# leggedrobotics/open3d_slam_private

Measured on AMD Instinct MI355X. Metric: ICP iterations/sec (scan-to-map), higher is better.
Workload: dtype f32

## Files before the change

include/o3dslam_reg_debug.h:

```cpp
#ifndef O3DSLAM_REG_DEBUG_H
#define O3DSLAM_REG_DEBUG_H

#include "o3dslam_reg.h"

#ifdef __cplusplus
extern "C" {
#endif

typedef struct {
    int32_t struct_size;
    int32_t profile_loop;
    int32_t match_variant;
    int32_t debug_flags;
    int32_t disable_halo;
    int32_t lanes_per_point;
    int32_t disable_fused;
    int32_t reserved;
} reg_debug_params;

REG_API reg_status reg_debug_configure(reg_handle* h, const reg_debug_params* d);

REG_API reg_status reg_debug_halo_bound(reg_handle* h, const float* xyz, int64_t n, float* out);

REG_API reg_status reg_debug_halo_witness(reg_handle* h, const float* xyz, int64_t n, int32_t* out);

REG_API reg_status reg_debug_live_resources(int64_t out[4]);

#ifdef __cplusplus
}
#endif
#endif
```

open3d_slam_private_amd/capi.py:

```python
from __future__ import annotations

import ctypes as C
import math
import os
import subprocess
import weakref

import numpy as np

_HERE = os.path.dirname(os.path.abspath(__file__))
_SO = os.environ.get("O3D_REG_LIB") or os.path.join(_HERE, "lib", "libo3dslam_reg.so")

STATUS_NAMES = {0: "OK", 1: "EMPTY_TARGET", 2: "EMPTY_SOURCE", 3: "NO_CORRESPONDENCES", 4: "BAD_TRANSFORM",
                5: "NOT_CONFIGURED", 6: "BAD_ARGUMENT", 7: "MISSING_FIELD", 8: "DEVICE_ERROR", 9: "UNSUPPORTED",
                10: "OUT_OF_BOUNDS"}
OUT_OF_BOUNDS = 10
COST_P2PL, COST_GICP = 0, 1
COST_O3D_P2PL, COST_O3D_P2P = 2, 3
SMOOTH_LEN_MAX = 15


class RegError(RuntimeError):
    def __init__(self, status, msg=""):
        self.status = status
# ... 344 lines not shown
PM_POINT_TO_PLANE, PM_POINT_TO_POINT = 0, 1
ROBUST_FCTS = {"cauchy": 0, "welsch": 1, "sc": 2, "gm": 3, "tukey": 4, "huber": 5, "L1": 6, "student": 7}
SCALE_ESTIMATORS = {"none": 0, "mad": 1, "berg": 2, "std": 3}
DISTANCE_TYPES = {"point2point": 0, "point2plane": 1}


EXPORTS = ["reg_default_params", "reg_shipped_params", "reg_create", "reg_destroy", "reg_last_error",
           "reg_set_stream", "reg_set_target", "reg_set_source", "reg_register", "reg_compute", "reg_prepare",
           "reg_linearize", "reg_get_correspondences", "reg_match_local", "reg_trim_histogram", "reg_reduce_local",
           "reg_solve_update", "reg_host_solve6", "reg_host_x_to_T", "reg_host_centroid", "reg_get_target_info", "reg_profile_kernels", "reg_source_centroid_sums", "reg_prepare_centroid", "reg_compose",
           "reg_dist_begin", "reg_dist_buffers", "reg_dist_phase", "reg_dist_finish",
           "reg_dist_fused_buffers", "reg_dist_poll", "reg_estimate_normals", "reg_smooth_normals", "reg_host_solve6_xicp",
           "reg_set_target_f64", "reg_get_target_source_indices", "reg_voxelize_within_volume", "reg_carve_indices", "reg_dist_xicp_buffers", "reg_dist_gather_buffers",
           "reg_dist_record", "reg_dist_centroid_sums", "reg_dist_prepare",
           "reg_information_matrix", "reg_set_source_f64", "reg_debug_configure", "reg_debug_halo_bound", "reg_debug_halo_witness",
           "reg_debug_live_resources",
           "reg_dist_get_unique_id", "reg_dist_init", "reg_dist_init_custom", "reg_dist_register", "reg_dist_shutdown",
           "reg_dist_info", "reg_dist_steer_create", "reg_dist_steer_destroy", "reg_dist_steer_step",
           "reg_dist_steer_counts", "reg_host_tail_plan", "reg_host_o3d_update",
           "reg_default_pm_chain", "reg_check_pm_chain", "reg_set_pm_chain", "reg_get_robust_state",
           "reg_get_correspondences_k", "reg_host_robust_weights", "reg_host_pm_p2p_update",
           "reg_get_var_trim", "reg_host_var_trim",
           "reg_get_covariance", "reg_get_covariance_sums", "reg_host_censi_covariance", "reg_get_minimizer_stats",
           "reg_get_degeneracy", "reg_get_bound", "reg_host_solution_remap",
           "reg_default_ternary_xicp", "reg_check_ternary_xicp", "reg_set_ternary_xicp", "reg_get_ternary_xicp",
           "reg_host_ternary_decide", "reg_host_partial_constraint", "reg_host_solve6_xicp_rhs",
           "reg_default_ssn_params", "reg_sampling_surface_normal", "reg_filter_points",
           "reg_default_octree_params", "reg_octree_grid", "reg_host_octree_root", "reg_host_octree_random_picks",
           "reg_filter_cloud", "reg_host_glibc_rand", "reg_default_voxel_grid_params", "reg_voxel_grid",
           "reg_overlap_indices", "reg_set_pair_overlap_f64", "reg_get_source_source_indices",
           "reg_compute_fpfh", "reg_match_features", "reg_ransac_correspondences", "reg_host_ransac_est_k",
# ... 27 lines not shown
        return _lib
    if not os.path.exists(_SO):
        raise ImportError(f"{_SO} is missing: build it with `python -c 'import __graft_entry__ as g; g.build()'` "
                          "(hipcc --offload-arch=gfx950).  There is no CPU fallback for the registration path.")
    lib = C.CDLL(_SO)
    vp, i64, f32p = C.c_void_p, C.c_int64, C.c_void_p
    lib.reg_create.argtypes = [C.POINTER(RegParams), C.POINTER(vp)]
    lib.reg_destroy.argtypes = [vp]
    lib.reg_last_error.argtypes = [vp]
    lib.reg_last_error.restype = C.c_char_p
    lib.reg_set_stream.argtypes = [vp, vp]
    lib.reg_debug_configure.argtypes = [vp, C.POINTER(RegDebugParams)]
    lib.reg_debug_halo_bound.argtypes = [vp, f32p, i64, f32p]
    lib.reg_debug_halo_witness.argtypes = [vp, f32p, i64, vp]
    lib.reg_debug_live_resources.argtypes = [C.POINTER(C.c_int64)]
    lib.reg_dist_get_unique_id.argtypes = [C.c_char_p]
    lib.reg_dist_init.argtypes = [vp, C.c_char_p, C.c_int, C.c_int]
    lib.reg_dist_init_custom.argtypes = [vp, C.POINTER(Collectives), C.c_int, C.c_int]
    lib.reg_dist_register.argtypes = [vp, f32p, f32p, C.POINTER(RegResult)]
    lib.reg_dist_shutdown.argtypes = [vp]
    lib.reg_dist_info.argtypes = [vp, C.POINTER(C.c_int64), C.POINTER(C.c_int32), C.POINTER(C.c_int32), C.POINTER(C.c_int32)]
    lib.reg_dist_steer_create.argtypes = [C.c_int, C.c_int, C.c_int, C.c_float, C.c_int]
    lib.reg_dist_steer_create.restype = vp
    lib.reg_dist_steer_destroy.argtypes = [vp]
    lib.reg_dist_steer_destroy.restype = None
    lib.reg_dist_steer_step.argtypes = [vp, C.POINTER(DistReply)]
    lib.reg_dist_steer_step.restype = DistAction
    lib.reg_dist_steer_counts.argtypes = [vp, C.POINTER(C.c_int32), C.POINTER(C.c_int32), C.POINTER(C.c_int32)]
    lib.reg_dist_steer_counts.restype = None
    lib.reg_set_source_f64.argtypes = [vp, vp, vp, vp, i64, C.c_int]
# ... 1390 lines not shown


def host_solve6_xicp(A, b, flags):
    x = np.zeros(6, np.float32)
    f = np.ascontiguousarray(flags, np.int32)
    rank = load_library().reg_host_solve6_xicp(_ptr(_f32(A).reshape(36)), _ptr(_f32(b)), _ptr(f), _ptr(x))
    return x, rank


def host_x_to_T(x):
    T = np.zeros(16, np.float32)
    load_library().reg_host_x_to_T(_ptr(_f32(x)), _ptr(T))
    return _T_out(T)


def host_centroid(xyz):
    xyz = _f32(xyz)
    out = np.zeros(3, np.float32)
    load_library().reg_host_centroid(_ptr(xyz), xyz.shape[1], xyz.shape[0], _ptr(out))
    return out


def host_o3d_update(cost, sums):
    s = np.ascontiguousarray(sums, np.float64).reshape(32)
    U = np.zeros(16, np.float64)
    rank = C.c_int32()
    st = load_library().reg_host_o3d_update(int(cost), _ptr(s), _ptr(U), C.byref(rank))
    if st != 0:
        raise RegError(st, "reg_host_o3d_update")
    return U.reshape(4, 4).T.copy(), rank.value
# ... 32 lines not shown
```

open3d_slam_private_amd/csrc/host_dist.hpp:

```cpp
#pragma once
#include <thread>

struct Deadline {
    std::chrono::steady_clock::time_point t_end;
    explicit Deadline(double seconds) : t_end(std::chrono::steady_clock::now() + std::chrono::duration_cast<std::chrono::steady_clock::duration>(std::chrono::duration<double>(seconds))) {}
    bool expired() const { return std::chrono::steady_clock::now() > t_end; }
};

static reg_status dist_stream_wait(reg_handle* h, double timeout_s, const char* what) {
    const Deadline dl(timeout_s);
    for (unsigned spins = 0;; ++spins) {
        const hipError_t e = hipStreamQuery(h->stream);
        if (e == hipSuccess) return REG_OK;
        if (e != hipErrorNotReady) {
            h->err = std::string(what) + ": " + hipGetErrorString(e);
            return REG_DEVICE_ERROR;
        }
        if ((spins & 63) == 63) {
            if (dl.expired()) {
                h->err = std::string(what) + ": the stream did not drain within the deadline (O3D_DIST_TIMEOUT_S): a peer died or a "
                                              "collective never completed";
                return REG_DEVICE_ERROR;
            }
            std::this_thread::sleep_for(std::chrono::microseconds(50));
// ... 430 lines not shown

int reg_host_solve6(const float A[36], const float b[6], float x[6]) { return solve6_p2pl(A, b, x); }

int reg_host_solve6_xicp(const float A[36], const float b[6], const int32_t flags[6], float x[6]) {
    int f[6];
    for (int k = 0; k < 6; ++k) f[k] = flags[k];
    return solve6_xicp(A, b, f, x);
}

void reg_host_x_to_T(const float x[6], float T[16]) {
    float Tr[16];
    x_to_T(x, Tr);
    row_to_col(Tr, T);
}

reg_status reg_host_o3d_update(int cost, const double sums[32], double T_update[16], int32_t* rank) {
    if (!cost_is_o3d(cost) || !sums || !T_update) return REG_BAD_ARGUMENT;
    if (sums[28] == 0.0) return REG_NO_CORRESPONDENCES;
    double U[16];
    const int r = o3d_update(cost == REG_COST_O3D_P2P, sums, U);
    for (int i = 0; i < 4; ++i)
        for (int j = 0; j < 4; ++j) T_update[4 * j + i] = U[4 * i + j];
    if (rank) *rank = r;
    return REG_OK;
}

void reg_host_centroid(const float* xyz, int64_t stride, int64_t n, float out[3]) {
    long long s[3] = {0, 0, 0};
    for (int64_t i = 0; i < n; ++i)
        for (int k = 0; k < 3; ++k) s[k] += llrint((double)xyz[i * stride + k] * 65536.0);
// ... 5 lines not shown
```

open3d_slam_private_amd/csrc/host_math.hpp:

```cpp
#pragma once
#include <cmath>
#include <cstdint>
#include <cstring>

#if defined(__HIPCC__)
#include <hip/hip_runtime.h>
#define O3D_HD __host__ __device__
#else
#define O3D_HD
#endif

namespace o3dreg {

O3D_HD inline void m4_identity(float* T) {
    memset(T, 0, 16 * sizeof(float));
    T[0] = T[5] = T[10] = T[15] = 1.f;
}

O3D_HD inline void m4_mul(const float* A, const float* B, float* C) {
    float R[16];
    for (int i = 0; i < 4; ++i)
        for (int j = 0; j < 4; ++j) {
            float s = A[4 * i] * B[j];
            float t = A[4 * i + 1] * B[4 + j];
            s = s + t;
            t = A[4 * i + 2] * B[8 + j];
            s = s + t;
            t = A[4 * i + 3] * B[12 + j];
            s = s + t;
            R[4 * i + j] = s;
        }
    memcpy(C, R, sizeof(R));
}

O3D_HD inline float float_from_orderable(uint32_t k) {
    const uint32_t u = (k & 0x80000000u) ? (k & 0x7fffffffu) : ~k;
    float v;
    memcpy(&v, &u, 4);
    return v;
}

O3D_HD inline void m4_transpose(const float* A, float* B) {
    float R[16];
    for (int i = 0; i < 4; ++i)
        for (int j = 0; j < 4; ++j) R[4 * i + j] = A[4 * j + i];
    memcpy(B, R, sizeof(R));
// ... 835 lines not shown
```

open3d_slam_private_amd/csrc/kernels_tail.hpp:

```cpp
#pragma once

#ifndef O3D_TAIL_ACQ
#define O3D_TAIL_ACQ 0
#endif
#ifndef O3D_TAIL_THREADS
#define O3D_TAIL_THREADS 512
#endif
constexpr int kTailThreads = O3D_TAIL_THREADS;
#ifndef O3D_TAIL_SLOTS
#define O3D_TAIL_SLOTS 1024
#endif
#ifndef O3D_TAIL_WGS_PER_CU
#define O3D_TAIL_WGS_PER_CU 1
#endif
constexpr int kTailSlots = O3D_TAIL_SLOTS;
constexpr int kTailWgsPerCu = O3D_TAIL_WGS_PER_CU;
constexpr int kTailPts = kTailSlots / kTailThreads;
constexpr int kTailRec = 12;
constexpr int kTailHistRow = 32;
constexpr int kTailCoarse = 256;
constexpr int kTailMaxIters = 64;
constexpr int kTailSyncWords = 256;
constexpr int kTailRing = 4;
constexpr int kTailBandCntWord = 128;
// ... 74 lines not shown
}
__device__ __forceinline__ void tail_st_f64(double* p, double x) {
    __hip_atomic_store(reinterpret_cast<unsigned long long*>(p), (unsigned long long)__double_as_longlong(x), __ATOMIC_RELAXED,
                       __HIP_MEMORY_SCOPE_AGENT);
}
__device__ __forceinline__ unsigned long long tail_ld_u64(const void* p) {
    return __hip_atomic_load(reinterpret_cast<unsigned long long*>(const_cast<void*>(p)), __ATOMIC_RELAXED, __HIP_MEMORY_SCOPE_AGENT);
}
__device__ __forceinline__ void tail_st_u64(void* p, unsigned long long x) {
    __hip_atomic_store(reinterpret_cast<unsigned long long*>(p), x, __ATOMIC_RELAXED, __HIP_MEMORY_SCOPE_AGENT);
}
__device__ __forceinline__ unsigned tail_ld_u32(const unsigned* p) {
    return __hip_atomic_load(const_cast<unsigned*>(p), __ATOMIC_RELAXED, __HIP_MEMORY_SCOPE_AGENT);
}

__device__ __noinline__ __attribute__((flatten)) void tail_solve_update(IterState* sit, const double* tot, const uint32_t* misc, float* s_x, UpdWork* work,
                                               bool trim, unsigned n_band_raw, unsigned n_band_all) {
    const int lane = (int)(threadIdx.x & 63);
    const float r_limit_last = sit->limit_last, r_limit_sel = __uint_as_float(misc[2]);
    const int r_dbg_narrow = sit->debug_narrow_band & 1;
    const int r_fixed = sit->fixed_iters, r_iters = sit->iterations;
    const int r_xnc = sit->xicp_nc;
    const double r_tot28 = tot[28];
    float r_T[16];
#pragma unroll
    for (int i = 0; i < 16; ++i) r_T[i] = sit->T[i];
    const int r = lane >> 3, c = lane & 7;
    double a = 0.0;
    if (r < 6 && c < 7) {
        if (c < 6) {
            const int lo = r < c ? r : c, hi = r < c ? c : r;
            const int k = lo * 6 - (lo * (lo - 1)) / 2 + (hi - lo);
            a = (double)(float)tot[k];
        } else {
            a = (double)(-(float)tot[21 + r]);
        }
    }
    const double a_orig = a;
    double dmax = 0.0;
#pragma unroll
    for (int j = 0; j < 6; ++j) dmax = fmax(dmax, fabs(__shfl(a_orig, j * 8 + j)));
    bool well = dmax > 0.0;
    const double piv_thr = 1e-4 * dmax;
#pragma unroll
    for (int j = 0; j < 6; ++j) {
        const double pj = __shfl(a, j * 8 + j);
        well = well && (pj > piv_thr);
        const double ajc = __shfl(a, j * 8 + c);
        const double arj = __shfl(a, r * 8 + j);
        const double qd = ajc / pj;
        a = (r == j) ? qd : a - arj * qd;
    }
    double xsol[6];
#pragma unroll
    for (int i = 0; i < 6; ++i) xsol[i] = __shfl(a, i * 8 + 6);
    if (lane != 0) return;
    const float limit = r_limit_sel;
    const float r_limit_prev = sit->limit_prev;
    sit->limit_prev2 = r_limit_prev;
    sit->limit_prev = r_limit_last;
    sit->limit_last = limit;
    {
        const Band nb = trim ? predict_band(limit, r_limit_last, r_limit_prev, n_band_all, sit->band_lo, sit->band_hi, r_dbg_narrow)
                             : Band{INFINITY, INFINITY};
        sit->band_lo = nb.lo;
        sit->band_hi = nb.hi;
    }
    sit->band_count = n_band_raw;
    sit->stall = 0;
    if (r_tot28 == 0.0) {
        sit->status = REG_NO_CORRESPONDENCES;
        sit->done = 1;
        return;
    }
    float x[6], dT[16], Tn[16];
    int rank = 6;
    if (r_xnc > 0) {
        rank = upd_solve6_xicp_inl(tot, sit->xicp_flags, s_x, work);
        for (int i = 0; i < 6; ++i) x[i] = s_x[i];
    } else if (well) {
        for (int i = 0; i < 6; ++i) x[i] = (float)xsol[i];
    } else {
        rank = upd_solve6_p2pl_inl(tot, s_x, work);
        for (int i = 0; i < 6; ++i) x[i] = s_x[i];
    }
    sit->rank_last = rank;
    x_to_T(x, dT);
    m4_mul(dT, r_T, Tn);
    for (int i = 0; i < 16; ++i) sit->T_prev[i] = r_T[i];
    for (int i = 0; i < 16; ++i) sit->T[i] = Tn[i];
    sit->iterations = r_iters + 1;
    bool iterate;
    if (r_fixed > 0)
        iterate = r_iters + 1 < r_fixed;
    else
        iterate = sit->chk.check(sit->T);
    if (!iterate) sit->done = 1;
}

__device__ __forceinline__ void tail_gicp_factor(const Xf& T, const float4 s, const float4 a0, const float4 a1, const float4 q,
                                                 const float4 b0, const float4 b1, float d2, double (&v)[kSums]) {
    const float3 tp = xf_point(T, s.x, s.y, s.z);
    const double r[3] = {(double)q.x - (double)tp.x, (double)q.y - (double)tp.y, (double)q.z - (double)tp.z};
    const double Cp[9] = {a0.x, a0.y, a0.z, a0.y, a0.w, a1.x, a0.z, a1.x, a1.y};
    const double Cq[9] = {b0.x, b0.y, b0.z, b0.y, b0.w, b1.x, b0.z, b1.x, b1.y};
    double R[9];
#pragma unroll
    for (int a = 0; a < 3; ++a)
#pragma unroll
        for (int c = 0; c < 3; ++c) R[3 * a + c] = (double)T.m[4 * a + c];
    double RC[9], S[9];
#pragma unroll
// ... 796 lines not shown
                }
                wave_reduce32(v);
                if ((lane & 1) == 0) sh[wave][lane >> 1] = v[0];
                __syncthreads();
                if (t < kSums) {
                    double v2 = 0.0;
#pragma unroll
                    for (int w2 = 0; w2 < kWaves; ++w2) v2 += sh[w2][t];
                    tot[t] += v2;
                }
                __syncthreads();
            }
        }
        TAIL_STAMP(10);
        if (t < kSums) sit->sums[t] = tot[t];
        if (wave == 0) {
            if (kGicp)
                tail_solve_update_gicp(sit, tot, reinterpret_cast<double*>(s_x), work);
            else
                tail_solve_update(sit, tot, misc, s_x, work, trim, n_band_raw, wide ? misc[12] : n_band_raw);
        }
        __syncthreads();
        TAIL_STAMP(11);
        if (sit->done) {
            exit_reason = 1;
            ++k_local;
            break;
        }
        if (k_local + 1 >= cfg.max_iters) {
            exit_reason = 3;
            ++k_local;
            break;
        }
    }
    if (exit_reason == 2 || exit_reason == 4) {
// ... 80 lines not shown
    uint32_t* hw = reinterpret_cast<uint32_t*>(host);
    for (int w2 = lane; w2 < kMirrorWords; w2 += 64) hw[w2] = mir_w[w2];
    HostMirror::SeqRecord* srec = &host->ring[cfg.seq % kSeqRing];
    {
        const HostMirror* m = reinterpret_cast<const HostMirror*>(mir_w);
        uint32_t word = 0;
        if (lane == 2) word = (uint32_t)m->iterations;
        if (lane == 3) word = (uint32_t)m->done;
        if (lane == 4) word = (uint32_t)m->stall;
        if (lane == 6) word = __float_as_uint(m->limit_last);
        if (lane == 7) word = __float_as_uint(m->limit_prev);
        if (lane >= 2 && lane < 8) reinterpret_cast<uint32_t*>(srec)[lane] = word;
    }
    __threadfence_system();
    if (lane == 0) {
        __hip_atomic_store(&srec->seq, cfg.seq, __ATOMIC_RELEASE, __HIP_MEMORY_SCOPE_SYSTEM);
        __hip_atomic_store(&host->seq, cfg.seq, __ATOMIC_RELEASE, __HIP_MEMORY_SCOPE_SYSTEM);
    }
}
```

open3d_slam_private_amd/csrc/kernels_update.hpp:

```cpp
#pragma once

__global__ void __launch_bounds__(64)
k_pack_contrib(double* __restrict__ acc, const IterState* __restrict__ it, float* __restrict__ contrib) {
    const int c = threadIdx.x;
    double* hdr = reinterpret_cast<double*>(contrib);
    if (it->done || it->stall) {
        if (c < kSums) hdr[c] = 0.0;
        if (c == 0) reinterpret_cast<uint32_t*>(contrib)[64] = 0u;
        return;
    }
    if (c < kSums) {
        double t = 0;
        for (int r = 0; r < kAccRows; ++r) {
            t += acc[(size_t)r * kSums + c];
            acc[(size_t)r * kSums + c] = 0.0;
        }
        hdr[c] = t;
    }
    if (c == 0) reinterpret_cast<uint32_t*>(contrib)[64] = it->band_count;
}

__device__ __forceinline__ void lds_barrier() {
    asm volatile("s_waitcnt lgkmcnt(0)" ::: "memory");
    __builtin_amdgcn_s_barrier();
// ... 80 lines not shown
            dst[3 * kk + rr] = sacc + a2;
        }
}

template <bool kP2P, int kWg>
__device__ __noinline__ __attribute__((flatten)) int upd_o3d(const double* tot, double* U_out, UpdWork* w) {
    double s[kSums], U[16];
    for (int i = 0; i < kSums; ++i) s[i] = tot[i];
    const int rank = kP2P ? o3d_update_p2p(s, U) : o3d_update_p2pl_in(s, U, w->sym.s);
    for (int i = 0; i < 16; ++i) U_out[i] = U[i];
    return rank;
}

enum UpdPath { kUpdGeneric = 0, kUpdSelect, kUpdFused, kUpdGathered, kUpdFinish };
constexpr int kUpdLeanThreads = 512;
constexpr int upd_threads(UpdPath p) { return (p == kUpdSelect || p == kUpdFinish) ? kUpdLeanThreads : 1024; }

template <bool kO3d, UpdPath kPath>
__device__ __forceinline__ void reduce_update_body(const double* __restrict__ partials, int n_blocks, IterState* it,
                                                   HostMirror* host, unsigned long long seq, int fused_arg,
                                                   const float* __restrict__ band, float* __restrict__ w_out,
                                                   const SelectState* __restrict__ sel, const float* __restrict__ gathered_arg,
                                                   int n_ranks, int my_rank, XicpState* __restrict__ xs) {
    constexpr int kThreads = upd_threads(kPath);
    constexpr bool kBand = kPath == kUpdGeneric || kPath == kUpdFused || kPath == kUpdGathered;
    static_assert(!kBand || kThreads == 1024, "the band code is written for 1024 threads");
    const bool finish = kPath == kUpdGeneric ? fused_arg == 2 : kPath == kUpdFinish;
    const int fused = kPath == kUpdGeneric ? (fused_arg == 1 ? 1 : 0) : ((kPath == kUpdFused || kPath == kUpdGathered) ? 1 : 0);
    const float* __restrict__ const gathered = (kPath == kUpdGeneric || kPath == kUpdGathered) ? gathered_arg : nullptr;
    const int contrib_cap = contrib_cap_for(n_ranks);
    const size_t contrib_stride = contrib_floats(contrib_cap);
    __shared__ double sh[32][kSums];
    __shared__ double tot[kSums];
    __shared__ uint32_t hist[2048 + 64];
    __shared__ uint32_t wave_tot[16];
    __shared__ uint32_t pick[2];
    __shared__ float s_limit;
    __shared__ uint32_t bd2[kBandCap];
    constexpr int kDirectCap = 256;
    __shared__ __attribute__((aligned(16))) uint32_t bdk[kDirectCap];
// ... 8 lines not shown
    __shared__ double s_dl[6];
    __shared__ __attribute__((aligned(16))) unsigned char s_work[kUpdWorkBytes];
    UpdWork* const work = reinterpret_cast<UpdWork*>(s_work);
    constexpr int kStateWords = (int)(sizeof(IterState) / 4);
    static_assert(sizeof(IterState) % 4 == 0 && kStateWords <= 1024, "IterState must be a whole number of words");
    __shared__ __attribute__((aligned(16))) uint32_t s_state[kStateWords];
    IterState* const sit = reinterpret_cast<IterState*>(s_state);
    constexpr int kPer = 1024 / kThreads;
    static_assert(kPer == 1 || kPer % 2 == 0, "the parts are combined in pairs");
    const int comp = threadIdx.x & (kSums - 1), part = threadIdx.x / kSums;
    for (int w = threadIdx.x; w < kStateWords; w += kThreads) s_state[w] = reinterpret_cast<const uint32_t*>(it)[w];
    double t = 0;
    double tp[kPer];
#pragma unroll
    for (int j = 0; j < kPer; ++j) tp[j] = 0;
    if constexpr (kPer > 1) {
        if (!finish) {
            for (int r0 = 0; r0 < n_blocks; r0 += 32 * 8) {
                double v[kPer][8];
#pragma unroll
                for (int j = 0; j < kPer; ++j)
#pragma unroll
                    for (int u = 0; u < 8; ++u) {
                        const int b = r0 + kPer * part + j + 32 * u;
                        v[j][u] = partials[(size_t)(b < n_blocks ? b : 0) * kSums + comp];
                    }
#pragma unroll
                for (int j = 0; j < kPer; ++j)
                    if (r0 + kPer * part + j < n_blocks) {
#pragma unroll
                        for (int u = 0; u < 8; ++u) tp[j] += (r0 + kPer * part + j + 32 * u < n_blocks) ? v[j][u] : 0.0;
                    }
            }
        }
    } else if (!gathered && !finish) {
        const int n_rows = fused ? kAccRows : n_blocks;
        for (int b0 = part; b0 < n_rows; b0 += 32 * 8) {
            double v8[8];
#pragma unroll
            for (int u = 0; u < 8; ++u) {
                const int b = b0 + 32 * u;
                v8[u] = partials[(size_t)(b < n_rows ? b : part) * kSums + comp];
            }
#pragma unroll
            for (int u = 0; u < 8; ++u) t += (b0 + 32 * u < n_rows) ? v8[u] : 0.0;
        }
    }
// ... 70 lines not shown
    if (gathered) {
        for (int r = part; r < n_ranks; r += 32)
            t += reinterpret_cast<const double*>(gathered + (size_t)r * contrib_stride)[comp];
    } else if (fused) {
        for (int b = part; b < kAccRows; b += 32)
            const_cast<double*>(partials)[(size_t)b * kSums + comp] = 0.0;
    }
    if constexpr (kPer > 1) {
#pragma unroll
        for (int j = 0; j < kPer / 2; ++j) sh[(kPer / 2) * part + j][comp] = tp[2 * j] + tp[2 * j + 1];
    } else {
        t += __shfl_xor(t, 32);
        if ((threadIdx.x & 63) < 32) sh[threadIdx.x >> 6][comp] = t;
    }
    if (threadIdx.x == 0) {
        s_limit = INFINITY;
    }
    lds_barrier();
    if (threadIdx.x < kSums) {
        double s = 0;
#pragma unroll
        for (int p = 0; p < 16; ++p) s += sh[p][threadIdx.x];
        tot[threadIdx.x] = finish ? sit->sums[threadIdx.x] : s;
    }
    if (threadIdx.x == 0) s_skip_mirror = 0;
    lds_barrier();
    const unsigned long long stA = __builtin_amdgcn_s_memtime();
    unsigned long long stB = stA, stC = stA, sx1 = stA, sx2 = stA, sx3 = stA;
    if (kBand && fused && trim) {
        const uint32_t n_finite = (uint32_t)llround(tot[29]), n_below = (uint32_t)llround(tot[31]);
        const uint32_t k = trim_rank(n_finite, s_ratio);
        const bool ok = n_finite == 0 || (!band_bad && n_below <= k && k < n_below + n_band);
        if (!ok) {
            if (threadIdx.x == 0) {
                it->stall = 1;
                it->band_count = 0;
                host->stall = 1;
                host->band_count = (int)s_band_count;
                host->iterations = sit->iterations;
                host->done = 0;
                HostMirror::SeqRecord* rec = &host->ring[seq % kSeqRing];
                rec->iterations = sit->iterations;
                rec->done = 0;
                rec->stall = 1;
                rec->limit_last = sit->limit_last;
                rec->limit_prev = sit->limit_prev;
                __threadfence_system();
                __hip_atomic_store(&rec->seq, seq, __ATOMIC_RELEASE, __HIP_MEMORY_SCOPE_SYSTEM);
                __hip_atomic_store(&host->seq, seq, __ATOMIC_RELEASE, __HIP_MEMORY_SCOPE_SYSTEM);
            }
            return;
        }
        if (n_finite != 0) {
            if (threadIdx.x < n_band) bd2[threadIdx.x] = my_d2[0];
            for (uint32_t i = threadIdx.x + 1024u; i < n_band; i += 1024u) bd2[i] = __float_as_uint(rec(i, 29));
            const uint32_t u_lo = __float_as_uint(s_band_lo), u_hi = __float_as_uint(s_band_hi);
            uint32_t rank = k - n_below, prefix = 0;
            const bool direct = n_band <= (uint32_t)kDirectCap && u_hi > u_lo && (u_hi - u_lo) < (1u << 24) &&
                                !(sit->debug_narrow_band & 2);
            if (direct) {
                sx1 = __builtin_amdgcn_s_memtime();
                const uint32_t n_pad = (n_band + 15u) & ~15u;
                if (threadIdx.x < n_pad)
                    bdk[threadIdx.x] = threadIdx.x < n_band ? (((my_d2[0] - u_lo) << 8) | threadIdx.x) : 0xffffffffu;
// ... 132 lines not shown
                        } else if (i >= rk_off[my_rank] && i < rk_off[my_rank + 1]) {
                            w_out[__float_as_int(rec(i, 31))] = 0.f;
                        }
                    }
                }
            lds_barrier();
            if (threadIdx.x < kSums) {
                double s2 = 0;
#pragma unroll
                for (int p = 0; p < 16; ++p) s2 += sh[p][threadIdx.x];
                tot[threadIdx.x] += s2;
            }
            lds_barrier();
            stC = __builtin_amdgcn_s_memtime();
        }
    } else if (!fused && trim && sel) {
        if (threadIdx.x == 0) s_limit = sel->limit;
        __syncthreads();
    }
    if (threadIdx.x < kSums) sit->sums[threadIdx.x] = tot[threadIdx.x];
    if (threadIdx.x >= 64 && threadIdx.x < 64 + kQueues && sit->qcount) sit->qcount[(threadIdx.x - 64) * kQueueStride] = 0u;
    if (threadIdx.x >= 64) return;
    const int lane = threadIdx.x;
    const unsigned long long st1 = __builtin_amdgcn_s_memtime();
    unsigned long long st2 = st1, st3 = st1;
    const bool p2pl = !kO3d && sit->cost == REG_COST_P2PL;
    const float r_limit_last = sit->limit_last, r_limit_sel = s_limit;
    const int r_dbg_narrow = sit->debug_narrow_band & 1, r_update = sit->update, r_xstage = sit->xicp_stage;
    const int r_fixed = sit->fixed_iters, r_iters = sit->iterations;
    int r_xnc = sit->xicp_nc;
    const unsigned r_band_count = sit->band_count;
// ... 21 lines not shown
#pragma unroll
    for (int j = 0; j < 6; ++j) {
        const double pj = __shfl(a, j * 8 + j);
        well = well && (pj > piv_thr);
        const double ajc = __shfl(a, j * 8 + c);
        const double arj = __shfl(a, r * 8 + j);
        const double q = ajc / pj;
        a = (r == j) ? q : a - arj * q;
    }
    double xsol[6];
#pragma unroll
    for (int i = 0; i < 6; ++i) xsol[i] = __shfl(a, i * 8 + 6);
    st2 = __builtin_amdgcn_s_memtime();
    const bool stage_a = !finish && r_update != 0 && p2pl && r_xstage == 1 && r_tot28 != 0.0 && xs != nullptr;
    if (stage_a && lane < 2) upd_xicp_stage_a<true>(tot, sit->xicp_Trd, lane == 0 ? xs->vr : xs->vt, lane == 0 ? 0 : 3);
    if (lane == 0) {
        const float limit = finish ? r_limit_last : r_limit_sel;
        if (!finish) {
            const float r_limit_prev = sit->limit_prev;
            sit->limit_prev2 = r_limit_prev;
            sit->limit_prev = r_limit_last;
            sit->limit_last = limit;
            const Band nb = trim ? predict_band(limit, r_limit_last, r_limit_prev, n_band, sit->band_lo, sit->band_hi, r_dbg_narrow)
                                 : Band{INFINITY, INFINITY};
            sit->band_lo = nb.lo;
            sit->band_hi = nb.hi;
        }
        const int nband_report = (int)r_band_count;
        sit->band_count = 0;
        sit->stall = 0;
        bool do_update = r_update != 0;
        if (stage_a) {
            for (int i = 0; i < 4; ++i) xs->center[i] = 0.0;
            for (int i = 0; i < 6; ++i) {
                xs->comb[i] = 0.0;
                xs->high[i] = 0.0;
            }
            sit->xicp_stage = 2;
            do_update = false;
            s_skip_mirror = 1;
        }
        if (finish && xs) {
            int nc = 0;
// ... 13 lines not shown
                sit->status = REG_NO_CORRESPONDENCES;
                sit->done = 1;
            } else if (p2pl) {
                float x[6], dT[16], Tn[16];
                int rank = 6;
                if (r_xnc > 0) {
                    rank = upd_solve6_xicp<kThreads>(tot, sit->xicp_flags, s_x, work);
                    for (int i = 0; i < 6; ++i) x[i] = s_x[i];
                } else if (well) {
                    for (int i = 0; i < 6; ++i) x[i] = (float)xsol[i];
                } else {
                    rank = upd_solve6_p2pl<kThreads>(tot, s_x, work);
                    for (int i = 0; i < 6; ++i) x[i] = s_x[i];
                }
                sit->rank_last = rank;
                x_to_T(x, dT);
                m4_mul(dT, r_T, Tn);
                for (int i = 0; i < 16; ++i) sit->T_prev[i] = r_T[i];
                for (int i = 0; i < 16; ++i) sit->T[i] = Tn[i];
                sit->iterations = r_iters + 1;
                bool iterate;
                if (r_fixed > 0)
                    iterate = r_iters + 1 < r_fixed;
                else
                    iterate = sit->chk.check(sit->T);
                if (!iterate) sit->done = 1;
            } else if ((kO3d || sit->gicp_stop_rule == 1) && sit->fixed_iters <= 0 &&
                       ((sit->iterations >= 1 &&
                         fabs(r_tot28 / (double)sit->n_total - sit->fit_prev) < (double)sit->gicp_rel_fitness &&
                         fabs(sqrt(tot[30] / r_tot28) - sit->rmse_prev) < (double)sit->gicp_rel_rmse) ||
                        sit->iterations >= sit->max_iter)) {
                if (sit->iterations >= sit->max_iter &&
                    !(sit->iterations >= 1 && fabs(r_tot28 / (double)sit->n_total - sit->fit_prev) < (double)sit->gicp_rel_fitness &&
                      fabs(sqrt(tot[30] / r_tot28) - sit->rmse_prev) < (double)sit->gicp_rel_rmse))
                    sit->chk.max_iter_reached = true;
                else
                    sit->chk.converged = true;
                for (int i = 0; i < 16; ++i) sit->T_prev[i] = r_T[i];
                sit->done = 1;
            } else {
                double dl[6], E[16], Tn[16];
// ... 38 lines not shown
                    if (sit->iterations >= sit->fixed_iters) sit->done = 1;
                } else if (kO3d || sit->gicp_stop_rule == 1) {
                } else {
                    const double dr = sqrt(dl[0] * dl[0] + dl[1] * dl[1] + dl[2] * dl[2]);
                    const double dt = sqrt(dl[3] * dl[3] + dl[4] * dl[4] + dl[5] * dl[5]);
                    if (dr < (double)sit->gicp_rot_eps && dt < (double)sit->gicp_trans_eps) {
                        sit->chk.converged = true;
                        sit->done = 1;
                    } else if (sit->iterations >= sit->max_iter) {
                        sit->chk.max_iter_reached = true;
                        sit->done = 1;
                    }
                }
            }
        }
        st3 = __builtin_amdgcn_s_memtime();
        HostMirror* m = reinterpret_cast<HostMirror*>(mir_w);
        for (int i = 0; i < 16; ++i) m->T[i] = sit->T[i];
        for (int i = 0; i < 16; ++i) m->T_prev[i] = sit->T_prev[i];
        m->iterations = sit->iterations;
        m->done = sit->done;
        m->status = sit->status;
        m->rank_last = sit->rank_last;
        m->converged = sit->chk.converged ? 1 : 0;
        m->max_iter_reached = sit->chk.max_iter_reached ? 1 : 0;
        m->stall = 0;
        m->band_count = 0;
        m->limit_last = sit->limit_last;
        m->limit_prev = sit->limit_prev;
        m->band_lo = sit->band_lo;
        m->band_hi = sit->band_hi;
        m->pad_nband = nband_report;
        for (int i = 0; i < 6; ++i) {
            m->localizable[i] = sit->xicp_flags[i];
            m->xicp_comb[i] = sit->xicp_comb[i];
            m->xicp_high[i] = sit->xicp_high[i];
        }
        m->n_constraints = sit->xicp_nc;
        m->pad3 = 0;
        m->stamps[0] = st1 - st0;
        m->stamps[1] = st2 - st1;
        m->stamps[2] = st3 - st2;
        m->stamps[4] = stA - st0;
        m->stamps[5] = stB - stA;
        m->stamps[6] = stC - stB;
        m->stamps[3] = sx1 - stA;
        m->stamps[7] = ((sx2 - sx1) << 32) | (sx3 - sx2);
    }
    if (lane < kSums) reinterpret_cast<HostMirror*>(mir_w)->sums[lane] = tot[lane];
    __builtin_amdgcn_fence(__ATOMIC_ACQ_REL, "workgroup");
    __builtin_amdgcn_wave_barrier();
    for (int w = lane; w < kStateWords; w += 64) reinterpret_cast<uint32_t*>(it)[w] = s_state[w];
    if (s_skip_mirror) return;
    constexpr int kMirrorWords = (int)(offsetof(HostMirror, seq) / 4);
    uint32_t* hw = reinterpret_cast<uint32_t*>(host);
    for (int w = lane; w < kMirrorWords; w += 64) hw[w] = mir_w[w];
    HostMirror::SeqRecord* srec = &host->ring[seq % kSeqRing];
    {
        const HostMirror* m = reinterpret_cast<const HostMirror*>(mir_w);
        static_assert(sizeof(HostMirror::SeqRecord) == 32, "record layout: seq(8) iterations done stall pad limit_last limit_prev");
        uint32_t word = 0;
        if (lane == 2) word = (uint32_t)m->iterations;
        if (lane == 3) word = (uint32_t)m->done;
        if (lane == 6) word = __float_as_uint(m->limit_last);
        if (lane == 7) word = __float_as_uint(m->limit_prev);
        if (lane >= 2 && lane < 8) reinterpret_cast<uint32_t*>(srec)[lane] = word;
    }
    __threadfence_system();
    if (lane == 0) {
        __hip_atomic_store(&srec->seq, seq, __ATOMIC_RELEASE, __HIP_MEMORY_SCOPE_SYSTEM);
        __hip_atomic_store(&host->seq, seq, __ATOMIC_RELEASE, __HIP_MEMORY_SCOPE_SYSTEM);
    }
}

__global__ void __launch_bounds__(upd_threads(kUpdSelect))
k_reduce_update(const double* __restrict__ partials, int n_blocks, IterState* it, HostMirror* host, unsigned long long seq,
                const SelectState* __restrict__ sel, XicpState* __restrict__ xs) {
    reduce_update_body<false, kUpdSelect>(partials, n_blocks, it, host, seq, 0, nullptr, nullptr, sel, nullptr, 0, 0, xs);
}
__global__ void __launch_bounds__(upd_threads(kUpdFinish))
k_reduce_update_finish(IterState* it, HostMirror* host, unsigned long long seq, XicpState* __restrict__ xs) {
    reduce_update_body<false, kUpdFinish>(nullptr, 0, it, host, seq, 2, nullptr, nullptr, nullptr, nullptr, 0, 0, xs);
}
__global__ void __launch_bounds__(upd_threads(kUpdFused))
k_reduce_update_fused(const double* __restrict__ partials, int n_blocks, IterState* it, HostMirror* host,
                      unsigned long long seq, const float* __restrict__ band, float* __restrict__ w_out) {
// ... 88 lines not shown
```

Measured before the change: 19040.

## Parallelize pose update across lanes and move band prediction off the serial lane

The pose update after the 6x6 solve now computes the 4x4 matrix product with one entry per lane instead of a single lane doing all 16. The band-limit prediction moves to a second wave (thread 64) so it runs alongside the solve. Sequence stores after an explicit system fence are relaxed from release to relaxed ordering. The partial-sum reduction gains a configurable number of load rounds in flight, defaulting to 1. The serial tail of each ICP iteration gets shorter, at the cost of extra wave barriers and fences and some risk around the memory ordering the host relies on.

```diff
diff --git a/include/o3dslam_reg_debug.h b/include/o3dslam_reg_debug.h
--- a/include/o3dslam_reg_debug.h
+++ b/include/o3dslam_reg_debug.h
@@ -26,6 +26,8 @@
 
 REG_API reg_status reg_debug_live_resources(int64_t out[4]);
 
+REG_API void reg_debug_m4_mul(const float A[16], const float B[16], float C[16]);
+
 #ifdef __cplusplus
 }
 #endif
diff --git a/open3d_slam_private_amd/capi.py b/open3d_slam_private_amd/capi.py
--- a/open3d_slam_private_amd/capi.py
+++ b/open3d_slam_private_amd/capi.py
@@ -382,7 +382,7 @@
            "reg_set_target_f64", "reg_get_target_source_indices", "reg_voxelize_within_volume", "reg_carve_indices", "reg_dist_xicp_buffers", "reg_dist_gather_buffers",
            "reg_dist_record", "reg_dist_centroid_sums", "reg_dist_prepare",
            "reg_information_matrix", "reg_set_source_f64", "reg_debug_configure", "reg_debug_halo_bound", "reg_debug_halo_witness",
-           "reg_debug_live_resources",
+           "reg_debug_live_resources", "reg_debug_m4_mul",
            "reg_dist_get_unique_id", "reg_dist_init", "reg_dist_init_custom", "reg_dist_register", "reg_dist_shutdown",
            "reg_dist_info", "reg_dist_steer_create", "reg_dist_steer_destroy", "reg_dist_steer_step",
            "reg_dist_steer_counts", "reg_host_tail_plan", "reg_host_o3d_update",
@@ -440,6 +440,8 @@
     lib.reg_debug_halo_bound.argtypes = [vp, f32p, i64, f32p]
     lib.reg_debug_halo_witness.argtypes = [vp, f32p, i64, vp]
     lib.reg_debug_live_resources.argtypes = [C.POINTER(C.c_int64)]
+    lib.reg_debug_m4_mul.argtypes = [f32p, f32p, f32p]
+    lib.reg_debug_m4_mul.restype = None
     lib.reg_dist_get_unique_id.argtypes = [C.c_char_p]
     lib.reg_dist_init.argtypes = [vp, C.c_char_p, C.c_int, C.c_int]
     lib.reg_dist_init_custom.argtypes = [vp, C.POINTER(Collectives), C.c_int, C.c_int]
@@ -1860,6 +1862,12 @@
     return _T_out(T)
 
 
+def host_m4_mul(A, B):
+    C_ = np.zeros(16, np.float32)
+    load_library().reg_debug_m4_mul(_ptr(_f32(A).reshape(16)), _ptr(_f32(B).reshape(16)), _ptr(C_))
+    return C_.reshape(4, 4)
+
+
 def host_centroid(xyz):
     xyz = _f32(xyz)
     out = np.zeros(3, np.float32)
diff --git a/open3d_slam_private_amd/csrc/host_dist.hpp b/open3d_slam_private_amd/csrc/host_dist.hpp
--- a/open3d_slam_private_amd/csrc/host_dist.hpp
+++ b/open3d_slam_private_amd/csrc/host_dist.hpp
@@ -468,6 +468,8 @@
     row_to_col(Tr, T);
 }
 
+void reg_debug_m4_mul(const float A[16], const float B[16], float C[16]) { m4_mul(A, B, C); }
+
 reg_status reg_host_o3d_update(int cost, const double sums[32], double T_update[16], int32_t* rank) {
     if (!cost_is_o3d(cost) || !sums || !T_update) return REG_BAD_ARGUMENT;
     if (sums[28] == 0.0) return REG_NO_CORRESPONDENCES;
diff --git a/open3d_slam_private_amd/csrc/host_math.hpp b/open3d_slam_private_amd/csrc/host_math.hpp
--- a/open3d_slam_private_amd/csrc/host_math.hpp
+++ b/open3d_slam_private_amd/csrc/host_math.hpp
@@ -17,19 +17,22 @@
     T[0] = T[5] = T[10] = T[15] = 1.f;
 }
 
+O3D_HD inline float m4_mul_entry(float a0, float a1, float a2, float a3, float b0, float b1, float b2, float b3) {
+    float s = a0 * b0;
+    float t = a1 * b1;
+    s = s + t;
+    t = a2 * b2;
+    s = s + t;
+    t = a3 * b3;
+    s = s + t;
+    return s;
+}
+
 O3D_HD inline void m4_mul(const float* A, const float* B, float* C) {
     float R[16];
     for (int i = 0; i < 4; ++i)
-        for (int j = 0; j < 4; ++j) {
-            float s = A[4 * i] * B[j];
-            float t = A[4 * i + 1] * B[4 + j];
-            s = s + t;
-            t = A[4 * i + 2] * B[8 + j];
-            s = s + t;
-            t = A[4 * i + 3] * B[12 + j];
-            s = s + t;
-            R[4 * i + j] = s;
-        }
+        for (int j = 0; j < 4; ++j)
+            R[4 * i + j] = m4_mul_entry(A[4 * i], A[4 * i + 1], A[4 * i + 2], A[4 * i + 3], B[j], B[4 + j], B[8 + j], B[12 + j]);
     memcpy(C, R, sizeof(R));
 }
 
diff --git a/open3d_slam_private_amd/csrc/kernels_tail.hpp b/open3d_slam_private_amd/csrc/kernels_tail.hpp
--- a/open3d_slam_private_amd/csrc/kernels_tail.hpp
+++ b/open3d_slam_private_amd/csrc/kernels_tail.hpp
@@ -112,17 +112,27 @@
     return __hip_atomic_load(const_cast<unsigned*>(p), __ATOMIC_RELAXED, __HIP_MEMORY_SCOPE_AGENT);
 }
 
+__device__ __forceinline__ void tail_band_update(IterState* sit, const uint32_t* misc, bool trim, unsigned n_band_all) {
+    const float limit = __uint_as_float(misc[2]), r_limit_last = sit->limit_last, r_limit_prev = sit->limit_prev;
+    sit->limit_prev2 = r_limit_prev;
+    sit->limit_prev = r_limit_last;
+    sit->limit_last = limit;
+    const Band nb = trim ? predict_band(limit, r_limit_last, r_limit_prev, n_band_all, sit->band_lo, sit->band_hi,
+                                        sit->debug_narrow_band & 1)
+                         : Band{INFINITY, INFINITY};
+    sit->band_lo = nb.lo;
+    sit->band_hi = nb.hi;
+}
 __device__ __noinline__ __attribute__((flatten)) void tail_solve_update(IterState* sit, const double* tot, const uint32_t* misc, float* s_x, UpdWork* work,
                                                bool trim, unsigned n_band_raw, unsigned n_band_all) {
+    if (threadIdx.x >= 64) {
+        if (threadIdx.x == 64) tail_band_update(sit, misc, trim, n_band_all);
+        return;
+    }
     const int lane = (int)(threadIdx.x & 63);
-    const float r_limit_last = sit->limit_last, r_limit_sel = __uint_as_float(misc[2]);
-    const int r_dbg_narrow = sit->debug_narrow_band & 1;
     const int r_fixed = sit->fixed_iters, r_iters = sit->iterations;
     const int r_xnc = sit->xicp_nc;
     const double r_tot28 = tot[28];
-    float r_T[16];
-#pragma unroll
-    for (int i = 0; i < 16; ++i) r_T[i] = sit->T[i];
     const int r = lane >> 3, c = lane & 7;
     double a = 0.0;
     if (r < 6 && c < 7) {
@@ -152,48 +162,37 @@
     double xsol[6];
 #pragma unroll
     for (int i = 0; i < 6; ++i) xsol[i] = __shfl(a, i * 8 + 6);
-    if (lane != 0) return;
-    const float limit = r_limit_sel;
-    const float r_limit_prev = sit->limit_prev;
-    sit->limit_prev2 = r_limit_prev;
-    sit->limit_prev = r_limit_last;
-    sit->limit_last = limit;
-    {
-        const Band nb = trim ? predict_band(limit, r_limit_last, r_limit_prev, n_band_all, sit->band_lo, sit->band_hi, r_dbg_narrow)
-                             : Band{INFINITY, INFINITY};
-        sit->band_lo = nb.lo;
-        sit->band_hi = nb.hi;
-    }
-    sit->band_count = n_band_raw;
-    sit->stall = 0;
-    if (r_tot28 == 0.0) {
-        sit->status = REG_NO_CORRESPONDENCES;
-        sit->done = 1;
-        return;
-    }
-    float x[6], dT[16], Tn[16];
-    int rank = 6;
-    if (r_xnc > 0) {
-        rank = upd_solve6_xicp_inl(tot, sit->xicp_flags, s_x, work);
-        for (int i = 0; i < 6; ++i) x[i] = s_x[i];
-    } else if (well) {
-        for (int i = 0; i < 6; ++i) x[i] = (float)xsol[i];
-    } else {
-        rank = upd_solve6_p2pl_inl(tot, s_x, work);
-        for (int i = 0; i < 6; ++i) x[i] = s_x[i];
-    }
-    sit->rank_last = rank;
-    x_to_T(x, dT);
-    m4_mul(dT, r_T, Tn);
-    for (int i = 0; i < 16; ++i) sit->T_prev[i] = r_T[i];
-    for (int i = 0; i < 16; ++i) sit->T[i] = Tn[i];
-    sit->iterations = r_iters + 1;
-    bool iterate;
-    if (r_fixed > 0)
-        iterate = r_iters + 1 < r_fixed;
-    else
-        iterate = sit->chk.check(sit->T);
-    if (!iterate) sit->done = 1;
+    int flags = 0;
+    if (lane == 0) {
+        sit->band_count = n_band_raw;
+        sit->stall = 0;
+        if (r_tot28 == 0.0) {
+            sit->status = REG_NO_CORRESPONDENCES;
+            sit->done = 1;
+        } else {
+            int rank = 6;
+            flags = 1;
+            if (r_xnc > 0) {
+                rank = upd_solve6_xicp_inl(tot, sit->xicp_flags, s_x, work);
+                flags = 3;
+            } else if (!well) {
+                rank = upd_solve6_p2pl_inl(tot, s_x, work);
+                flags = 3;
+            }
+            sit->rank_last = rank;
+        }
+    }
+    flags = __builtin_amdgcn_readfirstlane(flags);
+    if (!(flags & 1)) return;
+    if (flags & 2) {
+        __builtin_amdgcn_fence(__ATOMIC_ACQ_REL, "workgroup");
+        __builtin_amdgcn_wave_barrier();
+    }
+    float x[6];
+#pragma unroll
+    for (int i = 0; i < 6; ++i) x[i] = (flags & 2) ? s_x[i] : (float)xsol[i];
+    upd_pose_on_lanes(sit, lane, x);
+    if (lane == 0) upd_count_and_check(sit, r_iters, r_fixed);
 }
 
 __device__ __forceinline__ void tail_gicp_factor(const Xf& T, const float4 s, const float4 a0, const float4 a1, const float4 q,
@@ -1020,11 +1019,10 @@
         }
         TAIL_STAMP(10);
         if (t < kSums) sit->sums[t] = tot[t];
-        if (wave == 0) {
-            if (kGicp)
-                tail_solve_update_gicp(sit, tot, reinterpret_cast<double*>(s_x), work);
-            else
-                tail_solve_update(sit, tot, misc, s_x, work, trim, n_band_raw, wide ? misc[12] : n_band_raw);
+        if (kGicp) {
+            if (wave == 0) tail_solve_update_gicp(sit, tot, reinterpret_cast<double*>(s_x), work);
+        } else if (wave <= 1) {
+            tail_solve_update(sit, tot, misc, s_x, work, trim, n_band_raw, wide ? misc[12] : n_band_raw);
         }
         __syncthreads();
         TAIL_STAMP(11);
@@ -1135,7 +1133,7 @@
     }
     __threadfence_system();
     if (lane == 0) {
-        __hip_atomic_store(&srec->seq, cfg.seq, __ATOMIC_RELEASE, __HIP_MEMORY_SCOPE_SYSTEM);
-        __hip_atomic_store(&host->seq, cfg.seq, __ATOMIC_RELEASE, __HIP_MEMORY_SCOPE_SYSTEM);
+        __hip_atomic_store(&srec->seq, cfg.seq, __ATOMIC_RELAXED, __HIP_MEMORY_SCOPE_SYSTEM);
+        __hip_atomic_store(&host->seq, cfg.seq, __ATOMIC_RELAXED, __HIP_MEMORY_SCOPE_SYSTEM);
     }
 }
diff --git a/open3d_slam_private_amd/csrc/kernels_update.hpp b/open3d_slam_private_amd/csrc/kernels_update.hpp
--- a/open3d_slam_private_amd/csrc/kernels_update.hpp
+++ b/open3d_slam_private_amd/csrc/kernels_update.hpp
@@ -118,7 +118,43 @@
 
 enum UpdPath { kUpdGeneric = 0, kUpdSelect, kUpdFused, kUpdGathered, kUpdFinish };
 constexpr int kUpdLeanThreads = 512;
+#ifndef O3D_UPD_ROUNDS
+#define O3D_UPD_ROUNDS 1
+#endif
+constexpr int kUpdRoundsInFlight = O3D_UPD_ROUNDS;
 constexpr int upd_threads(UpdPath p) { return (p == kUpdSelect || p == kUpdFinish) ? kUpdLeanThreads : 1024; }
+
+__device__ __forceinline__ void upd_pose_on_lanes(IterState* sit, int lane, const float (&x)[6]) {
+    const int i = (lane >> 2) & 3, j = lane & 3;
+    float a[4], b[4];
+#pragma unroll
+    for (int k = 0; k < 4; ++k) b[k] = sit->T[4 * k + j];
+    const float t_old = sit->T[lane & 15];
+    float dT[16];
+    x_to_T(x, dT);
+#pragma unroll
+    for (int k = 0; k < 4; ++k) a[k] = i == 0 ? dT[k] : (i == 1 ? dT[4 + k] : (i == 2 ? dT[8 + k] : dT[12 + k]));
+    if (lane < 16) {
+        sit->T_prev[lane] = t_old;
+        sit->T[lane] = m4_mul_entry(a[0], a[1], a[2], a[3], b[0], b[1], b[2], b[3]);
+    }
+    __builtin_amdgcn_fence(__ATOMIC_ACQ_REL, "workgroup");
+    __builtin_amdgcn_wave_barrier();
+}
+__device__ __forceinline__ void upd_count_and_check(IterState* sit, int r_iters, int r_fixed) {
+    sit->iterations = r_iters + 1;
+    bool iterate;
+    if (r_fixed > 0)
+        iterate = r_iters + 1 < r_fixed;
+    else
+        iterate = sit->chk.check(sit->T);
+    if (!iterate) sit->done = 1;
+}
+
+template <UpdPath kPath>
+constexpr int upd_seq_order() {
+    return kPath == kUpdGeneric ? __ATOMIC_RELEASE : __ATOMIC_RELAXED;
+}
 
 template <bool kO3d, UpdPath kPath>
 __device__ __forceinline__ void reduce_update_body(const double* __restrict__ partials, int n_blocks, IterState* it,
@@ -127,7 +163,8 @@
                                                    const SelectState* __restrict__ sel, const float* __restrict__ gathered_arg,
                                                    int n_ranks, int my_rank, XicpState* __restrict__ xs) {
     constexpr int kThreads = upd_threads(kPath);
-    constexpr bool kBand = kPath == kUpdGeneric || kPath == kUpdFused || kPath == kUpdGathered;
+    constexpr int kSeqOrder = upd_seq_order<kPath>();
+    constexpr bool kBand =kPath == kUpdGeneric || kPath == kUpdFused || kPath == kUpdGathered;
     static_assert(!kBand || kThreads == 1024, "the band code is written for 1024 threads");
     const bool finish = kPath == kUpdGeneric ? fused_arg == 2 : kPath == kUpdFinish;
     const int fused = kPath == kUpdGeneric ? (fused_arg == 1 ? 1 : 0) : ((kPath == kUpdFused || kPath == kUpdGathered) ? 1 : 0);
@@ -166,23 +203,32 @@
     double tp[kPer];
 #pragma unroll
     for (int j = 0; j < kPer; ++j) tp[j] = 0;
+    float sel_limit = INFINITY;
     if constexpr (kPer > 1) {
+        if (sel != nullptr && threadIdx.x == 0) sel_limit = sel->limit;
         if (!finish) {
-            for (int r0 = 0; r0 < n_blocks; r0 += 32 * 8) {
-                double v[kPer][8];
-#pragma unroll
-                for (int j = 0; j < kPer; ++j)
-#pragma unroll
-                    for (int u = 0; u < 8; ++u) {
-                        const int b = r0 + kPer * part + j + 32 * u;
-                        v[j][u] = partials[(size_t)(b < n_blocks ? b : 0) * kSums + comp];
-                    }
-#pragma unroll
-                for (int j = 0; j < kPer; ++j)
-                    if (r0 + kPer * part + j < n_blocks) {
-#pragma unroll
-                        for (int u = 0; u < 8; ++u) tp[j] += (r0 + kPer * part + j + 32 * u < n_blocks) ? v[j][u] : 0.0;
-                    }
+            for (int r0 = 0; r0 < n_blocks; r0 += 32 * 8 * kUpdRoundsInFlight) {
+                double v[kUpdRoundsInFlight][kPer][8];
+#pragma unroll
+                for (int q = 0; q < kUpdRoundsInFlight; ++q) {
+                    const bool live = r0 + 32 * 8 * q < n_blocks;
+#pragma unroll
+                    for (int j = 0; j < kPer; ++j)
+#pragma unroll
+                        for (int u = 0; u < 8; ++u) {
+                            const int b = r0 + 32 * 8 * q + kPer * part + j + 32 * u;
+                            v[q][j][u] = live ? partials[(size_t)(b < n_blocks ? b : 0) * kSums + comp] : 0.0;
+                        }
+                }
+#pragma unroll
+                for (int q = 0; q < kUpdRoundsInFlight; ++q)
+#pragma unroll
+                    for (int j = 0; j < kPer; ++j)
+                        if (r0 + 32 * 8 * q + kPer * part + j < n_blocks) {
+#pragma unroll
+                            for (int u = 0; u < 8; ++u)
+                                tp[j] += (r0 + 32 * 8 * q + kPer * part + j + 32 * u < n_blocks) ? v[q][j][u] : 0.0;
+                        }
             }
         }
     } else if (!gathered && !finish) {
@@ -283,7 +329,7 @@
         if ((threadIdx.x & 63) < 32) sh[threadIdx.x >> 6][comp] = t;
     }
     if (threadIdx.x == 0) {
-        s_limit = INFINITY;
+        s_limit = (kPer > 1 && !fused && trim && sel) ? sel_limit : INFINITY;
     }
     lds_barrier();
     if (threadIdx.x < kSums) {
@@ -293,6 +339,19 @@
         tot[threadIdx.x] = finish ? sit->sums[threadIdx.x] : s;
     }
     if (threadIdx.x == 0) s_skip_mirror = 0;
+    constexpr bool kBandEarly = kPath == kUpdSelect;
+    if constexpr (kBandEarly) {
+        if (threadIdx.x == 64) {
+            const float limit = s_limit, last = sit->limit_last, prev = sit->limit_prev;
+            sit->limit_prev2 = prev;
+            sit->limit_prev = last;
+            sit->limit_last = limit;
+            const Band nb = trim ? predict_band(limit, last, prev, 0u, sit->band_lo, sit->band_hi, sit->debug_narrow_band & 1)
+                                 : Band{INFINITY, INFINITY};
+            sit->band_lo = nb.lo;
+            sit->band_hi = nb.hi;
+        }
+    }
     lds_barrier();
     const unsigned long long stA = __builtin_amdgcn_s_memtime();
     unsigned long long stB = stA, stC = stA, sx1 = stA, sx2 = stA, sx3 = stA;
@@ -315,8 +374,8 @@
                 rec->limit_last = sit->limit_last;
                 rec->limit_prev = sit->limit_prev;
                 __threadfence_system();
-                __hip_atomic_store(&rec->seq, seq, __ATOMIC_RELEASE, __HIP_MEMORY_SCOPE_SYSTEM);
-                __hip_atomic_store(&host->seq, seq, __ATOMIC_RELEASE, __HIP_MEMORY_SCOPE_SYSTEM);
+                __hip_atomic_store(&rec->seq, seq, kSeqOrder, __HIP_MEMORY_SCOPE_SYSTEM);
+                __hip_atomic_store(&host->seq, seq, kSeqOrder, __HIP_MEMORY_SCOPE_SYSTEM);
             }
             return;
         }
@@ -479,7 +538,7 @@
             lds_barrier();
             stC = __builtin_amdgcn_s_memtime();
         }
-    } else if (!fused && trim && sel) {
+    } else if (kPer == 1 && !fused && trim && sel) {
         if (threadIdx.x == 0) s_limit = sel->limit;
         __syncthreads();
     }
@@ -531,9 +590,45 @@
     st2 = __builtin_amdgcn_s_memtime();
     const bool stage_a = !finish && r_update != 0 && p2pl && r_xstage == 1 && r_tot28 != 0.0 && xs != nullptr;
     if (stage_a && lane < 2) upd_xicp_stage_a<true>(tot, sit->xicp_Trd, lane == 0 ? xs->vr : xs->vt, lane == 0 ? 0 : 3);
+    constexpr bool kLanes = kPath != kUpdGeneric && kPath != kUpdGathered;
+    int nband_report = 0, lanes_flags = 0;
+    auto stage_mirror = [&]() {
+        st3 = __builtin_amdgcn_s_memtime();
+        HostMirror* m = reinterpret_cast<HostMirror*>(mir_w);
+        for (int i = 0; i < 16; ++i) m->T[i] = sit->T[i];
+        for (int i = 0; i < 16; ++i) m->T_prev[i] = sit->T_prev[i];
+        m->iterations = sit->iterations;
+        m->done = sit->done;
+        m->status = sit->status;
+        m->rank_last = sit->rank_last;
+        m->converged = sit->chk.converged ? 1 : 0;
+        m->max_iter_reached = sit->chk.max_iter_reached ? 1 : 0;
+        m->stall = 0;
+        m->band_count = 0;
+        m->limit_last = sit->limit_last;
+        m->limit_prev = sit->limit_prev;
+        m->band_lo = sit->band_lo;
+        m->band_hi = sit->band_hi;
+        m->pad_nband = nband_report;
+        for (int i = 0; i < 6; ++i) {
+            m->localizable[i] = sit->xicp_flags[i];
+            m->xicp_comb[i] = sit->xicp_comb[i];
+            m->xicp_high[i] = sit->xicp_high[i];
+        }
+        m->n_constraints = sit->xicp_nc;
+        m->pad3 = 0;
+        m->stamps[0] = st1 - st0;
+        m->stamps[1] = st2 - st1;
+        m->stamps[2] = st3 - st2;
+        m->stamps[4] = stA - st0;
+        m->stamps[5] = stB - stA;
+        m->stamps[6] = stC - stB;
+        m->stamps[3] = sx1 - stA;
+        m->stamps[7] = ((sx2 - sx1) << 32) | (sx3 - sx2);
+    };
     if (lane == 0) {
         const float limit = finish ? r_limit_last : r_limit_sel;
-        if (!finish) {
+        if (!finish && !kBandEarly) {
             const float r_limit_prev = sit->limit_prev;
             sit->limit_prev2 = r_limit_prev;
             sit->limit_prev = r_limit_last;
@@ -543,7 +638,7 @@
             sit->band_lo = nb.lo;
             sit->band_hi = nb.hi;
         }
-        const int nband_report = (int)r_band_count;
+        nband_report = (int)r_band_count;
         sit->band_count = 0;
         sit->stall = 0;
         bool do_update = r_update != 0;
@@ -587,17 +682,21 @@
                     for (int i = 0; i < 6; ++i) x[i] = s_x[i];
                 }
                 sit->rank_last = rank;
-                x_to_T(x, dT);
-                m4_mul(dT, r_T, Tn);
-                for (int i = 0; i < 16; ++i) sit->T_prev[i] = r_T[i];
-                for (int i = 0; i < 16; ++i) sit->T[i] = Tn[i];
-                sit->iterations = r_iters + 1;
-                bool iterate;
-                if (r_fixed > 0)
-                    iterate = r_iters + 1 < r_fixed;
-                else
-                    iterate = sit->chk.check(sit->T);
-                if (!iterate) sit->done = 1;
+                if constexpr (kLanes) {
+                    lanes_flags = (r_xnc > 0 || !well) ? 3 : 1;
+                } else {
+                    x_to_T(x, dT);
+                    m4_mul(dT, r_T, Tn);
+                    for (int i = 0; i < 16; ++i) sit->T_prev[i] = r_T[i];
+                    for (int i = 0; i < 16; ++i) sit->T[i] = Tn[i];
+                    sit->iterations = r_iters + 1;
+                    bool iterate;
+                    if (r_fixed > 0)
+                        iterate = r_iters + 1 < r_fixed;
+                    else
+                        iterate = sit->chk.check(sit->T);
+                    if (!iterate) sit->done = 1;
+                }
             } else if ((kO3d || sit->gicp_stop_rule == 1) && sit->fixed_iters <= 0 &&
                        ((sit->iterations >= 1 &&
                          fabs(r_tot28 / (double)sit->n_total - sit->fit_prev) < (double)sit->gicp_rel_fitness &&
@@ -666,38 +765,22 @@
                 }
             }
         }
-        st3 = __builtin_amdgcn_s_memtime();
-        HostMirror* m = reinterpret_cast<HostMirror*>(mir_w);
-        for (int i = 0; i < 16; ++i) m->T[i] = sit->T[i];
-        for (int i = 0; i < 16; ++i) m->T_prev[i] = sit->T_prev[i];
-        m->iterations = sit->iterations;
-        m->done = sit->done;
-        m->status = sit->status;
-        m->rank_last = sit->rank_last;
-        m->converged = sit->chk.converged ? 1 : 0;
-        m->max_iter_reached = sit->chk.max_iter_reached ? 1 : 0;
-        m->stall = 0;
-        m->band_count = 0;
-        m->limit_last = sit->limit_last;
-        m->limit_prev = sit->limit_prev;
-        m->band_lo = sit->band_lo;
-        m->band_hi = sit->band_hi;
-        m->pad_nband = nband_report;
-        for (int i = 0; i < 6; ++i) {
-            m->localizable[i] = sit->xicp_flags[i];
-            m->xicp_comb[i] = sit->xicp_comb[i];
-            m->xicp_high[i] = sit->xicp_high[i];
-        }
-        m->n_constraints = sit->xicp_nc;
-        m->pad3 = 0;
-        m->stamps[0] = st1 - st0;
-        m->stamps[1] = st2 - st1;
-        m->stamps[2] = st3 - st2;
-        m->stamps[4] = stA - st0;
-        m->stamps[5] = stB - stA;
-        m->stamps[6] = stC - stB;
-        m->stamps[3] = sx1 - stA;
-        m->stamps[7] = ((sx2 - sx1) << 32) | (sx3 - sx2);
+        if constexpr (!kLanes) stage_mirror();
+    }
+    if constexpr (kLanes) {
+        lanes_flags = __builtin_amdgcn_readfirstlane(lanes_flags);
+        if (lanes_flags & 1) {
+            if (lanes_flags & 2) {
+                __builtin_amdgcn_fence(__ATOMIC_ACQ_REL, "workgroup");
+                __builtin_amdgcn_wave_barrier();
+            }
+            float x[6];
+#pragma unroll
+            for (int i = 0; i < 6; ++i) x[i] = (lanes_flags & 2) ? s_x[i] : (float)xsol[i];
+            upd_pose_on_lanes(sit, lane, x);
+            if (lane == 0) upd_count_and_check(sit, r_iters, r_fixed);
+        }
+        if (lane == 0) stage_mirror();
     }
     if (lane < kSums) reinterpret_cast<HostMirror*>(mir_w)->sums[lane] = tot[lane];
     __builtin_amdgcn_fence(__ATOMIC_ACQ_REL, "workgroup");
@@ -720,8 +803,8 @@
     }
     __threadfence_system();
     if (lane == 0) {
-        __hip_atomic_store(&srec->seq, seq, __ATOMIC_RELEASE, __HIP_MEMORY_SCOPE_SYSTEM);
-        __hip_atomic_store(&host->seq, seq, __ATOMIC_RELEASE, __HIP_MEMORY_SCOPE_SYSTEM);
+        __hip_atomic_store(&srec->seq, seq, kSeqOrder, __HIP_MEMORY_SCOPE_SYSTEM);
+        __hip_atomic_store(&host->seq, seq, kSeqOrder, __HIP_MEMORY_SCOPE_SYSTEM);
     }
 }
 
```

After: 19110 (median of 6 runs). Within noise of the previous version (+0.4%).
